# uio-bmi/compairr

Measured on AMD Instinct MI355X. Metric: query sequences/sec for --matrix d=1, 10M-vs-10M CDR3aa, higher is better.
Workload: dtype u64; 1 GPU; synthetic 10M-vs-10M CDR3aa, d=1 substitutions only, V/J matched; queries_total=10000000, queries_this_gpu=10000000, reference_sequences=10000000, matrix_checksum=fc9769626ca2bcf2c84e8473864b8853

## Files before the change

compairr_amd/csrc/query_layout.hip:

```cpp
#include "context.h"
#include "kernels_sliced.h"

#include <hipcub/hipcub.hpp>

#include <algorithm>
#include <atomic>
#include <chrono>
#include <cstdio>
#include <cstdlib>
#include <cstring>
#include <thread>

using namespace cmpr;

namespace {

constexpr uint32_t MAXP = 1 + MAX_CLASS_RES;
constexpr uint32_t FOREIGN_SLICES_LOG2 = 12;

enum : uint32_t { VERR_OFFSETS = 1, VERR_LONG = 2, VERR_REP = 3, VERR_GENE = 4, VERR_COUNT = 5,
                  VERR_RESIDUE = 6, VERR_TOO_LONG = 7, VERR_OFFSETS0 = 8 };

struct SliceTot {
  uint32_t tiles, chunks, small, list;
// ... 55 lines not shown
  SliceTot *tot[MAXP], *pre[MAXP];
  uint32_t  tile0[MAXP], chunk0[MAXP], list0[MAXP], small0[MAXP];
  unsigned long long res0[MAXP];
  uint32_t *tfirst_g;
  uint64_t *h_tmp, *hins_tmp, *hdel_tmp;
  uint32_t *ck_tmp;
  struct QAux *aux;
  TileDesc *tiles;
  Chunk    *chunks;
  TileRef  *tile_refs;
  uint32_t *small_tiles, *chunk_work;
  uint32_t *qres, *qv, *qj, *qck;
  uint64_t *qgh, *qhins, *qhdel;
  uint16_t *qlen;
  QueryRec *qrec;
  uint32_t  ngroups;
  uint32_t  goff[MAX_GROUPS];
  uint32_t  gslices[MAX_GROUPS];
  uint32_t  gslice0[MAX_GROUPS];
  uint32_t  sub2_items;
  uint2    *slice_items;
  uint32_t  nitem_slices;
  uint32_t  cblocks;
  uint32_t *ccnt, *cbase, *cfill, *cnch, *cchpre;
  uint32_t *ccnt_r, *cfill_r, *rbase;
  uint32_t  item_reps;
  uint32_t  item_wg;
  uint32_t  recompute;
  uint32_t  total_on_device;
  uint32_t  zob_lds, zob_words;
  uint32_t  zob_pos_words;
  uint32_t  own_np;
  uint32_t  ctab_lds;
  uint32_t  group_wg, G;
  uint32_t *gbase_w;
  uint32_t  cchunk0;
  cmpr::ItemRec *items;
  cmpr::ResPack *cpk;
  uint32_t           *verr;
  double             *rep_total;
  unsigned long long *alg_bytes;
};

constexpr uint32_t ITEM_WG_MAX = 16384;
constexpr uint32_t ITEM_PAD = 16;
constexpr uint32_t GROUP_WG_MAX = 8192;

enum : uint32_t { LDBG_NO_RANK = 1u << 16, LDBG_NO_ITEM_COUNT = 1u << 17, LDBG_NO_HASH = 1u << 18,
                  LDBG_NO_TOTALS = 1u << 19, LDBG_NO_CLASSKEY = 1u << 20, LDBG_NO_TMP_WRITES = 1u << 21,
                  LDBG_S_NO_REC = 1u << 22, LDBG_S_NO_ITEMS = 1u << 23, LDBG_S_SEQ_REC = 1u << 24,
                  LDBG_S_NO_ITEM_WRITE = 1u << 25, LDBG_S_NO_BASE = 1u << 26 };
#ifdef CMPR_ABLATION
#define LDBG(Q, bit) (((Q).dbg & (bit)) != 0)
#else
#define LDBG(Q, bit) false
#endif

__device__ inline uint64_t total_of(const QL &Q)
{
  return Q.total_on_device ? Q.off[Q.n] : Q.total;
}

__host__ __device__ inline uint32_t work_owner(uint32_t slice, uint32_t pass, uint32_t step)
{
  return (uint32_t)((((uint64_t)slice * 2654435761u + pass * 40503u) >> 7) % step);
}
// ... 119 lines not shown
      } else {
        uint64_t lo = 0, hi = 0;
        for (uint32_t x = 0; x < 16u && at + x < total; x++) {
          const uint64_t r = Q.res[at + x];
          if (x < 8u)
            lo |= r << (8u * x);
          else
            hi |= r << (8u * (x - 8u));
        }
        o.w[k] = make_uint4((uint32_t)lo, (uint32_t)(lo >> 32), (uint32_t)hi, (uint32_t)(hi >> 32));
      }
    }
  }
  return o;
}

template <int NP>
__device__ inline const uint8_t *own_commit(const QL &Q, const OwnPieces<NP> &o, uint64_t b, uint64_t e, uint32_t *mine)
{
  if (!o.fits)
    return Q.res + b;
  const uint64_t a0 = b & ~15ull;
#pragma unroll
  for (uint32_t k = 0; k < (uint32_t)NP; k++)
    if (a0 + 16u * k < e) {
      mine[4 * k + 0] = o.w[k].x;
      mine[4 * k + 1] = o.w[k].y;
      mine[4 * k + 2] = o.w[k].z;
      mine[4 * k + 3] = o.w[k].w;
    }
  return (const uint8_t *)mine + (b - a0);
}

template <typename ZP>
__device__ inline void hashes_of(ZP z, uint32_t A, bool indels, const uint8_t *s, uint32_t L, uint64_t &h,
                                 uint64_t &hins, uint64_t &hdel)
{
  for (uint32_t p = 0; p < L; p++) {
    const uint32_t r = s[p];
    h ^= z[A * p + r];
    if (indels) {
      hins ^= z[A * (p + 1) + r];
      if (p > 0)
        hdel ^= z[A * (p - 1) + r];
    }
  }
}

__device__ inline uint64_t variants_of(const QL &Q, const uint8_t *s, uint32_t L)
{
  const uint64_t A = Q.A;
  uint64_t n = 1;
  if (Q.differences >= 1) {
    n += (A - 1) * L;
    if (Q.indels) {
      if (L > 1) {
        uint64_t runs = 1;
        for (uint32_t p = 1; p < L; p++)
          runs += s[p] != s[p - 1];
        n += runs;
      }
      n += A + (A - 1) * (uint64_t)L;
    }
  }
  if (Q.differences >= 2)
    n += (A - 1) * (A - 1) * (uint64_t)L * (L ? L - 1 : 0) / 2;
  return n;
}

enum : uint32_t { ITEM_SUB = K_SUB, ITEM_INS = K_INS, ITEM_SUB2 = K_SUB2, ITEM_PAIR = 7  };

__device__ inline uint32_t class_base_of(const QL &Q, uint64_t i)
{
  const uint32_t L = (uint32_t)(Q.off[i + 1] - Q.off[i]);
  return class_base(Q.geom.ctab, Q.geom, Q.genes != 0, L, Q.genes ? Q.v[i] : 0u,
                    Q.genes ? Q.j[i] : 0u);
}

template <bool HASH, typename F>
__device__ inline void for_each_item(const QL &Q, const uint32_t *ct, const uint64_t *zt, uint64_t h_of_q,
                                     uint64_t hins_of_q, const uint8_t *s, uint32_t L, uint32_t ck, bool heavy, F f)
{
  const SliceGeom &g = Q.geom;
  const uint32_t K = g.k, A = Q.A;
  if (L == 0 || K == 0 || Q.differences < 1)
    return;
  if (Q.sub2_items) {
    if (heavy && L >= g.c0 + K && L <= RESPACK_MAX)
      for (uint32_t ci = 0; ci < K; ci++) {
        const uint32_t pos = g.c0 + ci, r = s[pos];
        for (uint32_t kp = 1; kp < A; kp++) {
          const uint32_t v = (r + kp) % A;
          const uint32_t key = ck ^ ct[g.off_cr + ci * A + r] ^ ct[g.off_cr + ci * A + v];
          f((key & g.smask) * Q.ngroups + (ci * (A - 1) + kp - 1), 0ull, kp | (pos << 8) | (ITEM_SUB2 << 24));
        }
      }
    return;
  }
  if (Q.pairs) {
    if (heavy) {
      const uint64_t h = HASH ? h_of_q : 0ull;
      for (uint32_t ci = 0; ci < K; ci++) {
        const uint32_t p = class_pos(L, ci, g.c0) & ~1u;
        bool first = true;
        uint32_t key = ck;
        for (uint32_t k = 0; k < K; k++) {
          const uint32_t mk = class_pos(L, k, g.c0);
          if ((mk & ~1u) == p) {
            if (k < ci)
              first = false;
            key ^= ct[g.off_cr + k * A + s[mk]];
          }
        }
        if (first) {
          const uint32_t ra = s[p], rb = p + 1 < L ? (uint32_t)s[p + 1] : A;
          uint64_t w = 0;
          if (HASH) {
            w = h ^ zt[A * p + ra];
            if (p + 1 < L)
              w ^= zt[A * (p + 1) + rb];
          }
          uint32_t fl = 0;
          if (Q.indels && L > 1) {
            if (p == 0 || s[p] != s[p - 1])
              fl |= ITEM_DEL_COUNTS;
            if (p + 1 < L && s[p + 1] != s[p])
              fl |= ITEM_DEL2_COUNTS;
          }
          key ^= pair_part_terms(ct, g, A, L, p, [&](uint32_t pos) -> uint32_t { return s[pos]; });
          f(Q.goff[ci] + (key & g.cmask), w, ra | (rb << 5) | (p << 10) | (ITEM_PAIR << 24) | fl);
        }
      }
    }
    if (!Q.indels)
      return;
    uint32_t base = ck;
    if (heavy)
      for (uint32_t k = 0; k < K; k++)
        base ^= ct[g.off_cr + k * A + s[class_pos(L, k, g.c0)]];
    const uint32_t base_i = base ^ ct[L] ^ ct[L + 1];
    if (!class_is_heavy(g.ctab, g, base_i))
      return;
    const uint64_t hins = HASH ? hins_of_q : 0ull;
    uint64_t P0 = 0, Pp = 0;
    uint64_t cand = 0;
    bool cand_far = false;
    for (uint32_t k = 0; k < K; k++) {
      const uint32_t mk = class_pos(L + 1, k, g.c0);
      if (mk < 64u)
        cand |= 1ull << (mk & ~1u);
      else
        cand_far = true;
    }
    for (uint32_t x = 0; x <= L; x++) {
      if ((x & 1u) == 0 && (x < 64u ? ((cand >> x) & 1ull) != 0 : cand_far)) {
        int ci = -1;
        uint32_t key = base_i;
        for (uint32_t k = 0; k < K; k++) {
          const uint32_t mk = class_pos(L + 1, k, g.c0);
          if ((mk & ~1u) == x) {
            if (ci < 0)
              ci = (int)k;
          } else {
            key ^= ct[g.off_cr + k * A + s[mk < x ? mk : mk - 1]];
          }
        }
        if (ci >= 0) {
          key ^= pair_part_terms(ct, g, A, L + 1, x,
                                 [&](uint32_t pos) -> uint32_t { return s[pos < x ? pos : pos - 1]; });
          uint64_t w = P0 ^ hins ^ Pp;
          if (HASH && x < L)
            w ^= zt[A * (x + 1) + s[x]];
          f(Q.goff[ci] + (key & g.cmask), w,
            (x < L ? (uint32_t)s[x] : A) | ((x > 0 ? (uint32_t)s[x - 1] : 31u) << 5) | (x << 10) | (ITEM_INS << 24));
// ... 18 lines not shown
        if (class_pos(L, k, g.c0) == pos) {
          if (k < ci)
            first = false;
          key ^= ct[g.off_cr + k * A + s[pos]];
        }
      if (first)
        f(Q.goff[ci] + (key & g.cmask), HASH ? h ^ zt[A * pos + s[pos]] : 0ull,
          (uint32_t)s[pos] | (pos << 8) | (ITEM_SUB << 24));
    }
  }
}

template <int MODE>
__device__ inline void layout_mode_assume(const QL &Q)
{
  if (MODE == 3) {
    __builtin_assume(Q.own_np == 3);
    return;
  }
  if (MODE != 0) {
    __builtin_assume(Q.rows != 0);
    __builtin_assume(Q.pairs != 0);
    __builtin_assume(Q.sliced != 0);
    __builtin_assume(Q.pairs2 == 0);
    __builtin_assume(Q.sub2_items == 0);
    __builtin_assume(Q.direct == 0);
    __builtin_assume(Q.route == 0);
    __builtin_assume(Q.differences == 1);
    __builtin_assume(Q.recompute != 0);
    __builtin_assume(Q.wstep <= 1);
    __builtin_assume(Q.dbg == 0);
    __builtin_assume(Q.group_wg == 0);
    __builtin_assume(Q.own_np == 3);
  }
  if (MODE == 1)
    __builtin_assume(Q.indels == 0);
  if (MODE == 2)
    __builtin_assume(Q.indels != 0);
}

template <uint32_t LAYOUT_WG, int MODE>
__global__ void __launch_bounds__(LAYOUT_WG, (LAYOUT_WG == 1024 || MODE == 0) ? 4 : 6)
keys_kernel(const QL Q, uint64_t q0, uint64_t q1, uint32_t row0)
{
  layout_mode_assume<MODE>(Q);
  extern __shared__ double tot_lds[];
  __shared__ uint32_t dest_lds[64];
  const bool lds_tot = Q.n_rep <= 2048;
  uint64_t *const zl = (uint64_t *)(tot_lds + (lds_tot ? Q.n_rep : 0u));
  uint32_t *const ctl = (uint32_t *)(zl + (Q.zob_lds ? Q.zob_words : 0u));
  uint32_t *const ihist = ctl + (Q.ctab_lds ? Q.geom.off_hv : 0u);
  uint32_t *const ghist = ihist + (Q.item_wg ? Q.nitem_slices : 0u);
  constexpr int NP = MODE == 0 ? OWN_NP_MAX : 3;
  const uint32_t own_np = MODE == 0 ? Q.own_np : 3u, own_dw = 4u * own_np + 1u;
  uint32_t *const mine = ghist + (Q.group_wg ? Q.G : 0u) + threadIdx.x * own_dw;
  const uint32_t *const ct = Q.ctab_lds ? ctl : Q.geom.ctab;
  if (lds_tot) {
    for (uint32_t r = threadIdx.x; r < Q.n_rep; r += LAYOUT_WG)
      tot_lds[r] = 0.0;
  }
  if (Q.zob_lds)
    for (uint32_t k = threadIdx.x; k < Q.zob_words; k += LAYOUT_WG)
      zl[k] = Q.zob[k];
  if (Q.ctab_lds)
    for (uint32_t k = threadIdx.x; k < Q.geom.off_hv; k += LAYOUT_WG)
      ctl[k] = Q.geom.ctab[k];
  if (Q.item_wg)
    for (uint32_t k = threadIdx.x; k < Q.nitem_slices; k += LAYOUT_WG)
      ihist[k] = 0;
  if (Q.group_wg)
    for (uint32_t k = threadIdx.x; k < Q.G; k += LAYOUT_WG)
      ghist[k] = 0;
  if (threadIdx.x < 64)
    dest_lds[threadIdx.x] = 0;
  if (Q.total_on_device && blockIdx.x == 0 && threadIdx.x == 0 && q0 == 0 && Q.off[0] != 0)
    atomicCAS(Q.verr, 0u, (uint32_t)VERR_OFFSETS0);
  const uint64_t total = total_of(Q);
  __syncthreads();
  unsigned long long alg = 0;
  uint32_t err_all = 0, Lmax = 0;
  struct Fields {
    uint64_t b, e, cn;
    uint32_t rp, vg, jg;
  };
  auto fetch = [&](uint64_t i) -> Fields {
    Fields f;
    f.b = f.e = 0;
    f.cn = 1;
    f.rp = f.vg = f.jg = 0;
    if (i < q1) {
      f.b = Q.off[i];
      f.e = Q.off[i + 1];
      f.rp = Q.rep[i];
      if (Q.genes) {
        f.vg = Q.v[i];
        f.jg = Q.j[i];
      }
      if (Q.counts)
        f.cn = Q.cnt[i];
    }
    return f;
  };
  const uint64_t stride = (uint64_t)gridDim.x * LAYOUT_WG;
  uint64_t i = q0 + (uint64_t)blockIdx.x * LAYOUT_WG + threadIdx.x;
  Fields cur = fetch(i);
  uint64_t pend_i = ~0ull;
  uint32_t pend_rank = 0;
  for (; i < q1; i += stride) {
    uint32_t err = 0;
    const uint64_t b = cur.b, e = cur.e;
    uint32_t L = 0;
    if (e < b || e > total)
      err = VERR_OFFSETS;
    else if (e - b > 0xffffu)
      err = VERR_LONG;
    else if (e - b > Q.longest)
      err = VERR_TOO_LONG;
    else
      L = (uint32_t)(e - b);
    const uint32_t rp = cur.rp;
    if (!err && rp >= Q.n_rep)
      err = VERR_REP;
    if (!err && Q.genes && (cur.vg >= Q.n_v_max || cur.jg >= Q.n_j_max))
      err = VERR_GENE;
    if (!err && Q.counts && cur.cn < 1)
      err = VERR_COUNT;
    OwnPieces<NP> pieces;
    pieces.fits = false;
    if (!err)
      pieces = own_load<NP>(Q, b, e, total, own_np);
    const Fields nxt = fetch(i + stride);
    const uint8_t *s = err ? Q.res : own_commit(Q, pieces, b, e, mine);
    if (pend_i != ~0ull) {
      Q.rank[pend_i] = pend_rank;
      pend_i = ~0ull;
    }
    const uint64_t cnt_i = cur.cn;
    const uint32_t vg = cur.vg, jg = cur.jg;
    cur = nxt;
    if (!err) {
      bool bad = false;
      for (uint32_t p = 0; p < L; p++)
        bad = bad || s[p] >= Q.A;
      if (bad)
        err = VERR_RESIDUE;
    }
    uint32_t grp_out = 0xffffffffu;
    if (err && !err_all)
      err_all = err;
    if (!err) {
      Lmax = max(Lmax, L);
      const double x = Q.counts ? (double)cnt_i : 1.0;
      if (lds_tot)
        unsafeAtomicAdd(tot_lds + rp, x);
      else
        unsafeAtomicAdd(Q.rep_total + rp, x);
      uint32_t ck = 0;
      bool heavy = false;
      if (Q.sliced && !LDBG(Q, LDBG_NO_CLASSKEY)) {
        ck = class_base(ct, Q.geom, Q.genes != 0, L, vg, jg);
        heavy = Q.geom.k > 0 && class_is_heavy(Q.geom.ctab, Q.geom, ck);
        if (heavy && L > 0)
          for (uint32_t k = 0; k < Q.geom.k; k++)
            ck ^= ct[Q.geom.off_cr + k * Q.A + s[class_pos(L, k, Q.geom.c0)]];
      } else if (Q.sliced)
        ck = (uint32_t)i * 2654435761u;
      if (Q.rows || Q.direct) {
        uint64_t h = 0;
        if (Q.genes) {
          if (Q.zob_lds) {
            const uint64_t *gk = zl + Q.A * Q.zpos;
            h = gk[vg] ^ gk[Q.n_v + jg];
          } else {
            const uint64_t *gk = Q.zob + (uint64_t)Q.A * Q.zpos;
            h = gk[vg] ^ gk[Q.n_v + jg];
          }
        }
        uint64_t hins = h, hdel = h;
        if (Q.zob_lds)
          hashes_of((const uint64_t *)zl, Q.A, Q.indels != 0, s, LDBG(Q, LDBG_NO_HASH) ? 0u : L, h, hins, hdel);
        else
          hashes_of(Q.zob, Q.A, Q.indels != 0, s, LDBG(Q, LDBG_NO_HASH) ? 0u : L, h, hins, hdel);
        if (Q.direct) {
          ck = (uint32_t)(h >> 40);
          Q.h_tmp[i] = h;
        } else if (!LDBG(Q, LDBG_NO_TMP_WRITES)) {
          Q.h_tmp[i] = h;
          if (Q.indels) {
            Q.hins_tmp[i] = hins;
            Q.hdel_tmp[i] = hdel;
          }
          Q.ck_tmp[i] = ck;
        }
      } else if (Q.sub2_items) {
        Q.ck_tmp[i] = ck;
      }
      if (Q.route) {
        unsigned long long mask = 1ull << work_owner(Q.sliced ? (ck & Q.geom.smask) : (ck & DIRECT_OWNER_MASK), 0u, Q.wstep);
        if (Q.ngroups)
          for_each_item<false>(Q, ct, Q.zob, 0ull, 0ull, s, L, ck, heavy, [&](uint32_t k, uint64_t, uint32_t) {
            mask |= 1ull << item_owner(Q, k, Q.wstep);
          });
        if (Q.route == 2u)
          mask = Q.wstep >= 64u ? ~0ull : (1ull << Q.wstep) - 1ull;
        grp_out = (uint32_t)mask;
        Q.rank[i] = (uint32_t)(mask >> 32);
        for (unsigned long long m = mask; m; m &= m - 1ull)
          atomicAdd(&dest_lds[__builtin_ctzll(m)], 1u);
      }
      bool any_item = false;
      if (Q.ngroups && !Q.route && !LDBG(Q, LDBG_NO_ITEM_COUNT))
        for_each_item<false>(Q, ct, Q.zob, 0ull, 0ull, s, L, ck, heavy, [&](uint32_t k, uint64_t, uint32_t) {
          if (item_owned(Q, k)) {
            if (Q.item_wg)
              atomicAdd(&ihist[k], 1u);
            else
              atomicAdd(Q.ccnt_r + (size_t)((uint32_t)(i >> 8) % Q.item_reps) * Q.nitem_slices + k, 1u);
            any_item = true;
          }
        });
      const uint64_t gl = Q.longest - L;
      const uint32_t slice = Q.sliced ? (ck & Q.geom.smask) : (ck & Q.pmask);
      uint64_t bucket = ~0ull;
      if (owned(Q, Q.sliced ? slice : (ck & DIRECT_OWNER_MASK), 0u))
        bucket = Q.sliced ? 2 * (uint64_t)slice + (heavy ? 1 : 0) : slice;
      else if (any_item)
        bucket = 2 * (Q.nslices_real + (((uint32_t)i * 2654435761u) >> (32 - FOREIGN_SLICES_LOG2)));
      if (bucket != ~0ull && !Q.route) {
        const uint32_t g = (uint32_t)(bucket * Q.per_slice + gl);
        grp_out = g;
        pend_rank = (LDBG(Q, LDBG_NO_RANK) ? 0u : Q.group_wg ? atomicAdd(&ghist[g], 1u) : atomicAdd(Q.cnt_g[0] + g, 1u)) |
                    (heavy ? 0x80000000u : 0u);
        pend_i = i;
      }
      if (Q.alg_step <= 1u || work_owner(Q.sliced ? slice : (ck & DIRECT_OWNER_MASK), 0u, Q.alg_step) == Q.alg_first)
        alg += LDBG(Q, LDBG_NO_TOTALS) ? 0ull : (uint64_t)L + 20 + 8 * variants_of(Q, s, L);
    }
    Q.grp[0][i] = grp_out;
  }
  if (pend_i != ~0ull)
    Q.rank[pend_i] = pend_rank;
  if (err_all)
    atomicCAS(Q.verr, 0u, err_all);
  uint32_t m = Lmax;
  for (int o = 32; o > 0; o >>= 1)
    m = max(m, (uint32_t)__shfl_down((int)m, o, WAVE));
  if ((threadIdx.x & 63) == 0 && m)
    atomicMax(Q.verr + 1, m);
  for (int o = 32; o > 0; o >>= 1)
    alg += __shfl_down(alg, o, WAVE);
  if ((threadIdx.x & 63) == 0 && alg)
    atomicAdd(Q.alg_bytes, alg);
  __syncthreads();
  if (lds_tot) {
    for (uint32_t r = threadIdx.x; r < Q.n_rep; r += LAYOUT_WG)
      if (tot_lds[r] != 0.0)
        unsafeAtomicAdd(Q.rep_total + r, tot_lds[r]);
  }
  if (Q.route && threadIdx.x < 64 && dest_lds[threadIdx.x])
    atomicAdd(Q.dest_cnt + threadIdx.x, (unsigned long long)dest_lds[threadIdx.x]);
  if (Q.group_wg) {
    uint32_t *const row = Q.gbase_w + (size_t)(row0 + blockIdx.x) * Q.G;
    for (uint32_t g = threadIdx.x; g < Q.G; g += LAYOUT_WG) {
      const uint32_t cn = ghist[g];
      if (cn)
        row[g] = atomicAdd(Q.cnt_g[0] + g, cn);
    }
  }
  if (Q.item_wg) {
    uint32_t *const row = Q.rbase + (size_t)(row0 + blockIdx.x) * Q.nitem_slices;
    for (uint32_t k = threadIdx.x; k < Q.nitem_slices; k += LAYOUT_WG) {
      const uint32_t cn = ihist[k];
      if (cn)
        row[k] = atomicAdd(Q.ccnt_r + (size_t)k * ITEM_PAD, cn);
// ... 157 lines not shown
              ck.pass |= CHUNK_WITH_ITEMS;
            if (Q.pairs2) {
              uint32_t lmax = 0;
              for (uint32_t t = 0; t < ck.ntiles; t++)
                lmax = max(lmax, Q.tiles[tile_base + k * Q.chunk_tiles + t].len);
              ck.pass |= ((lmax + 1u) / 2u) << 16;
            }
            Q.chunks[Q.chunk0[pi] + at.chunks + k * reps + rp] = ck;
          }
      }
    }
  }
  if (!WRITE) {
    SliceTot t;
    t.tiles = ntiles;
    t.chunks = nchunks;
    t.small = nsmall;
    t.list = nlist;
    t.res = res;
    Q.tot[pi][sl] = t;
  }
  (void)work_lens;
}


template <uint32_t LAYOUT_WG, int MODE>
__global__ void __launch_bounds__(LAYOUT_WG, (LAYOUT_WG == 1024 || MODE == 0) ? 4 : 6)
scatter_kernel(const QL Q, uint64_t q0, uint64_t q1, uint32_t row0)
{
  layout_mode_assume<MODE>(Q);
  extern __shared__ uint64_t scat_lds[];
  uint64_t *const zl = scat_lds;
  uint32_t *const ctl = (uint32_t *)(zl + (Q.zob_lds ? Q.zob_pos_words : 0u));
  uint32_t *const ibase = ctl + (Q.ctab_lds ? Q.geom.off_hv : 0u);
  uint32_t *const gb = ibase + (Q.item_wg ? Q.nitem_slices : 0u);
  constexpr int NP = MODE == 0 ? OWN_NP_MAX : 3;
  const uint32_t own_np = MODE == 0 ? Q.own_np : 3u, own_dw = 4u * own_np + 1u;
  uint32_t *const wave_words = gb + (Q.group_wg ? Q.G : 0u) + (threadIdx.x & ~63u) * own_dw;
  const uint32_t lane = threadIdx.x & 63u;
  uint32_t *const mine = wave_words + lane * own_dw;
  const uint32_t *const ct = Q.ctab_lds ? ctl : Q.geom.ctab;
  const uint64_t *const zt = Q.zob_lds ? zl : Q.zob;
  if (Q.zob_lds)
    for (uint32_t k = threadIdx.x; k < Q.zob_pos_words; k += LAYOUT_WG)
      zl[k] = Q.zob[k];
  if (Q.ctab_lds)
    for (uint32_t k = threadIdx.x; k < Q.geom.off_hv; k += LAYOUT_WG)
      ctl[k] = Q.geom.ctab[k];
  if (Q.group_wg) {
    const uint32_t *const row = Q.gbase_w + (size_t)(row0 + blockIdx.x) * Q.G;
    for (uint32_t g = threadIdx.x; g < Q.G; g += LAYOUT_WG)
      gb[g] = Q.base_g[0][g] + row[g];
  }
  if (Q.zob_lds || Q.ctab_lds || Q.group_wg)
    __syncthreads();
  if (Q.item_wg) {
    const uint32_t *const row = Q.rbase + (size_t)(row0 + blockIdx.x) * Q.nitem_slices;
    for (uint32_t k = threadIdx.x; k < Q.nitem_slices; k += LAYOUT_WG)
      ibase[k] = Q.cbase[k] + row[k];
    __syncthreads();
  }
  const uint64_t total = total_of(Q);
  struct Fields {
    uint64_t b, e;
    uint32_t g, rk;
  };
  const bool want_h = Q.ngroups != 0 && Q.rows, want_ck = Q.ngroups != 0 && (Q.rows || Q.sub2_items);
  auto fetch = [&](uint64_t i) -> Fields {
    Fields f;
    f.b = f.e = 0;
    f.g = 0xffffffffu;
    f.rk = 0;
    if (i < q1) {
      f.g = Q.grp[0][i];
      f.rk = Q.rank[i];
      f.b = Q.off[i];
      f.e = Q.off[i + 1];
    }
    return f;
  };
// ... 5 lines not shown
    uint32_t slot = 0xffffffffu;
    QueryRec qr;
    qr.cnt = 0;
    qr.v = qr.j = qr.rep = qr.len = qr.orig = 0;
    const uint32_t g = cur.g;
    const uint64_t b = cur.b, e = cur.e;
    const uint32_t rk = cur.rk;
    uint32_t gbase = 0, ck = 0;
    uint64_t h_q = 0, hins_q = 0;
    OwnPieces<NP> pieces;
    pieces.fits = false;
    if (g != 0xffffffffu) {
      gbase = LDBG(Q, LDBG_S_NO_BASE) ? 0u : Q.group_wg ? gb[g] : Q.base_g[0][g];
      pieces = own_load<NP>(Q, b, e, total, own_np);
      qr.cnt = Q.counts ? Q.cnt[i] : 1ull;
      qr.v = Q.genes ? Q.v[i] : 0u;
      qr.j = Q.genes ? Q.j[i] : 0u;
      qr.orig = Q.orig ? Q.orig[i] : (uint32_t)i;
      qr.rep = Q.existence ? qr.orig : Q.rep[i];
      if (want_h) {
        h_q = Q.h_tmp[i];
        if (Q.indels)
          hins_q = Q.hins_tmp[i];
      }
      if (want_ck)
        ck = Q.ck_tmp[i];
      if (Q.rec_hash && !want_h)
        h_q = Q.h_tmp[i];
    }
    cur = fetch(i + stride);
    if (g != 0xffffffffu) {
      slot = LDBG(Q, LDBG_S_NO_BASE) ? (uint32_t)i : gbase + (rk & 0x7fffffffu);
      const uint32_t L = (uint32_t)(e - b);
      const uint8_t *s = own_commit(Q, pieces, b, e, mine);
      qr.len = L;
      if (!Q.recompute) {
        QAux a;
        a.h = a.hins = a.hdel = 0;
        a.ck = 0;
        a.src = (uint32_t)i;
        if (Q.rows) {
          a.h = Q.h_tmp[i];
          a.ck = Q.ck_tmp[i];
          if (Q.indels) {
            a.hins = Q.hins_tmp[i];
            a.hdel = Q.hdel_tmp[i];
          }
        } else if (Q.direct) {
          a.h = Q.h_tmp[i];
        } else if (Q.genes) {
          const uint64_t *gk = Q.zob + (uint64_t)Q.A * Q.zpos;
          a.h = gk[Q.v[i]] ^ gk[Q.n_v + Q.j[i]];
        }
        Q.aux[slot] = a;
      }
      if (Q.ngroups != 0 && !LDBG(Q, LDBG_S_NO_ITEMS)) {
        const bool heavy = (rk >> 31) != 0;
        uint64_t hq = 0;
        cmpr::ResPack pk{};
        if (Q.pairs2 && heavy)
          for (uint32_t x = 0; x < L && x < RESPACK_MAX; x++)
            pk.w[x >> 4] |= ((uint32_t)s[x] & 3u) << ((x & 15u) * 2u);
        if (Q.sub2_items && heavy && L <= RESPACK_MAX) {
          if (Q.genes) {
            const uint64_t *gk = Q.zob + (uint64_t)Q.A * Q.zpos;
            hq = gk[qr.v] ^ gk[Q.n_v + qr.j];
          }
          for (uint32_t x = 0; x < L; x++) {
            const uint32_t r = s[x];
            hq ^= Q.zob[Q.A * x + r];
            pk.w[x >> 4] |= (r & 3u) << ((x & 15u) * 2u);
          }
        }
        for_each_item<true>(Q, ct, zt, h_q, hins_q, s, L, ck, heavy, [&](uint32_t k, uint64_t w, uint32_t crp) {
          if (!item_owned(Q, k))
            return;
          uint32_t item;
          if (Q.item_wg) {
            item = atomicAdd(&ibase[k], 1u);
          } else {
            const size_t rk = (size_t)((uint32_t)(i >> 8) % Q.item_reps) * Q.nitem_slices + k;
            item = Q.cbase[k] + Q.rbase[rk] + atomicAdd(Q.cfill_r + rk, 1u);
          }
          if (Q.sub2_items) {
            w = hq;
            Q.cpk[item] = pk;
          } else if (Q.pairs2) {
            Q.cpk[item] = pk;
          }
          ItemRec it;
          it.w = w;
          it.main = slot;
          it.rp = crp;
          if (!LDBG(Q, LDBG_S_NO_ITEM_WRITE))
            Q.items[item] = it;
        });
      }
    }
    if (slot != 0xffffffffu) {
      const uint32_t L = (uint32_t)(e - b);
      if (pieces.fits) {
        const uint32_t o = (uint32_t)(b & 15u), w0 = o >> 2, sh = o & 3u;
        uint32_t lo = mine[w0];
#pragma unroll
        for (uint32_t w = 0; w < 9; w++) {
          const uint32_t hi = mine[w0 + w + 1u];
          const uint32_t d = __builtin_amdgcn_alignbyte(hi, lo, sh);
// ... 909 lines not shown
  c->npasses = 1 + ngroups;
  const uint64_t chunk_tiles =
      c->chunk_tiles > 0 ? (uint64_t)c->chunk_tiles : c->rows ? 64 : 8 * (uint64_t)c->waves_per_block;
  c->chunk_cap = (uint32_t)chunk_tiles;
  const bool mixed_ok = c->sliced && (!c->opt.indels || c->rows);
  const uint64_t n2s = indel_passes ? 2 * nslices : 0;

  struct Range { uint64_t q0, q1; uint32_t grid, row0; };
  std::vector<Range> ranges;
  const bool item_wg = ncs > 0 && ncs <= ITEM_WG_MAX && !routing && c->item_wg != 0;
  const uint64_t zob_words = (uint64_t)A * c->zpos + (c->opt.ignore_genes ? 0 : c->opt.n_v_genes + c->opt.n_j_genes);
  const bool zob_lds = c->layout_zob_lds != 0 && zob_words * sizeof(uint64_t) <= 12288;
  const uint64_t zob_pos_words = (uint64_t)A * c->zpos;
  const bool ctab_lds = c->layout_zob_lds != 0 && c->sliced && c->geom.off_hv <= 2048;
  const size_t ctab_bytes = ctab_lds ? (size_t)c->geom.off_hv * sizeof(uint32_t) : 0;
  const uint32_t own_np_want = std::min<uint32_t>((uint32_t)OWN_NP_MAX, std::max<uint32_t>(3u, (Lcap + 15u + 15u) / 16u));
  const bool group_wg = G <= GROUP_WG_MAX && !routing && c->item_wg != 0;
  const size_t keys_shared = (n_rep <= 2048 ? n_rep * sizeof(double) : 0) + (zob_lds ? zob_words * sizeof(uint64_t) : 0) +
                             ctab_bytes + (item_wg ? (size_t)ncs * sizeof(uint32_t) : 0) + (group_wg ? G * sizeof(uint32_t) : 0);
  const size_t scatter_shared = (zob_lds ? zob_pos_words * sizeof(uint64_t) : 0) + ctab_bytes +
                                (item_wg ? (size_t)ncs * sizeof(uint32_t) : 0) + (group_wg ? G * sizeof(uint32_t) : 0);
  typedef void (*LayoutFn)(const QL, uint64_t, uint64_t, uint32_t);
  static const uint32_t wg_sizes[3] = {256, 512, 1024};
  static const LayoutFn keys_all[4][3] = {{keys_kernel<256, 0>, keys_kernel<512, 0>, keys_kernel<1024, 0>},
                                          {keys_kernel<256, 1>, keys_kernel<512, 1>, keys_kernel<1024, 1>},
                                          {keys_kernel<256, 2>, keys_kernel<512, 2>, keys_kernel<1024, 2>},
                                          {keys_kernel<256, 3>, keys_kernel<512, 3>, keys_kernel<1024, 3>}};
  static const LayoutFn scatter_all[4][3] = {{scatter_kernel<256, 0>, scatter_kernel<512, 0>, scatter_kernel<1024, 0>},
                                             {scatter_kernel<256, 1>, scatter_kernel<512, 1>, scatter_kernel<1024, 1>},
                                             {scatter_kernel<256, 2>, scatter_kernel<512, 2>, scatter_kernel<1024, 2>},
                                             {scatter_kernel<256, 3>, scatter_kernel<512, 3>, scatter_kernel<1024, 3>}};
  const bool recompute_on = Lcap <= 36u && !c->d2pairs && c->layout_recompute != 0;
  const int lmode = (c->rows && pair_rows(c) && !c->d2pairs && !sub2_items && !direct && !routing && wstep <= 1 &&
                     c->opt.differences == 1 && recompute_on && c->debug == 0 && !group_wg)
                        ? (c->opt.indels ? 2 : 1)
                        : own_np_want == 3u ? 3 : 0;
  const LayoutFn *const keys_fns = keys_all[lmode], *const scatter_fns = scatter_all[lmode];
  const uint32_t own_np = lmode ? 3u : own_np_want;
  uint32_t resident = 2048;
  uint32_t LAYOUT_WG = 256;
  size_t keys_lds = 0, scatter_lds = 0;
  LayoutFn keys_fn = keys_fns[0], scatter_fn = scatter_fns[0];
  {
    uint32_t best_waves = 0;
    int bk = 0, bs = 0;
    for (int w = 0; w < 3; w++) {
      const size_t own = (size_t)wg_sizes[w] * (4 * own_np + 1) * sizeof(uint32_t);
      const size_t kl = keys_shared + own, sl = scatter_shared + own;
      if (kl > 160 * 1024 - 512 || sl > 160 * 1024 - 512)
        continue;
      if ((rc = raise_lds_limit(c, (const void *)keys_fns[w], kl))) return rc;
      if ((rc = raise_lds_limit(c, (const void *)scatter_fns[w], sl))) return rc;
      const int ok = occupancy_of(c, (const void *)keys_fns[w], (int)wg_sizes[w], kl);
      const int os = occupancy_of(c, (const void *)scatter_fns[w], (int)wg_sizes[w], sl);
      const uint32_t waves = (uint32_t)std::max(0, std::min(ok, os)) * wg_sizes[w] / WAVE;
      if (waves >= best_waves && waves > 0) {
        best_waves = waves;
        LAYOUT_WG = wg_sizes[w];
        keys_lds = kl;
        scatter_lds = sl;
        keys_fn = keys_fns[w];
        scatter_fn = scatter_fns[w];
        resident = (uint32_t)c->cus * (uint32_t)std::min(ok, os);
        bk = ok;
        bs = os;
      }
    }
    if (best_waves == 0)
      return fail(c, CMPR_EUNSUPPORTED, "the layout kernels' tables do not fit the 160 KiB LDS");
    if (getenv("COMPAIRR_HIP_DEBUG"))
      fprintf(stderr, "compairr_hip: layout kernels: workgroups of %u; keys %zu B of LDS, %d per CU; scatter %zu B, %d; "
                      "grid %u; %llu item counters in %u groups (%s)\n", LAYOUT_WG, keys_lds, bk, scatter_lds, bs,
              resident, (unsigned long long)ncs, ngroups, item_wg ? "per workgroup in LDS" : "replicas in memory");
  }
  {
    const uint64_t min_range = 1u << 18;
    const uint64_t nr = from_host ? std::max<uint64_t>(1, std::min<uint64_t>(4, n / min_range)) : 1;
    static const uint32_t cut4[5] = {0, 30, 60, 86, 100};
    uint32_t row = 0;
    for (uint64_t r = 0; r < nr; r++) {
      Range g;
      g.q0 = nr == 4 ? n * cut4[r] / 100 : n * r / nr;
      g.q1 = nr == 4 ? n * cut4[r + 1] / 100 : n * (r + 1) / nr;
      g.grid = (uint32_t)std::min<uint64_t>(std::max<uint64_t>(1, (g.q1 - g.q0 + LAYOUT_WG - 1) / LAYOUT_WG), resident);
      g.row0 = row;
      row += g.grid;
      ranges.push_back(g);
    }
  }
  const uint64_t item_rows = (uint64_t)ranges.back().row0 + ranges.back().grid;

  ArenaCut cut;
  const size_t o_gcnt = cut.take(G * npass * sizeof(uint32_t));
  const uint32_t item_reps = item_wg ? ITEM_PAD : ncs > 0 && ncs <= 65536 ? 32u : 1u;
  const size_t o_ccnt = cut.take(ncs * sizeof(uint32_t));
  const size_t o_cfill = cut.take(ncs * sizeof(uint32_t));
  const size_t o_ccnt_r = cut.take(ncs * item_reps * sizeof(uint32_t));
  const size_t o_cfill_r = cut.take(item_wg ? 0 : ncs * item_reps * sizeof(uint32_t));
  const size_t o_sibcnt = cut.take(n2s * sizeof(uint32_t));
  const size_t o_sibfill = cut.take(n2s * sizeof(uint32_t));
  const size_t o_alg = cut.take(sizeof(unsigned long long));
  const size_t o_verr = cut.take(2 * sizeof(uint32_t));
  const size_t o_reptot = cut.take((size_t)n_rep * sizeof(double));
  const size_t o_dest = cut.take(2 * 64 * sizeof(unsigned long long));
  const size_t o_sums = cut.take(8 * sizeof(unsigned long long));
  const size_t zero_bytes = cut.used;
// ... 152 lines not shown
  Q.hdel_tmp = (uint64_t *)at(o_hdel);
  Q.ck_tmp = (uint32_t *)at(o_ck);
  Q.alg_bytes = (unsigned long long *)at(o_alg);
  Q.verr = (uint32_t *)at(o_verr);
  Q.rep_total = (double *)at(o_reptot);
  Q.ccnt = (uint32_t *)at(o_ccnt);
  Q.cbase = (uint32_t *)at(o_cbase);
  Q.cfill = (uint32_t *)at(o_cfill);
  Q.ccnt_r = (uint32_t *)at(o_ccnt_r);
  Q.cfill_r = (uint32_t *)at(o_cfill_r);
  Q.rbase = (uint32_t *)at(o_rbase);
  Q.item_reps = item_reps;
  Q.item_wg = item_wg ? 1u : 0u;
  Q.group_wg = group_wg ? 1u : 0u;
  Q.G = (uint32_t)G;
  Q.gbase_w = (uint32_t *)at(o_gbase_w);
  Q.recompute = recompute_on ? 1u : 0u;
  Q.total_on_device = total_on_device ? 1u : 0u;
  Q.cnch = (uint32_t *)at(o_cnch);
  Q.cchpre = (uint32_t *)at(o_cchpre);
  uint32_t *const cpad = (uint32_t *)at(o_cpad);
  uint32_t *const sib_cnt = (uint32_t *)at(o_sibcnt), *const sib_fill = (uint32_t *)at(o_sibfill);
  uint32_t *const sib_nch = (uint32_t *)at(o_sibnch), *const sib_lpre = (uint32_t *)at(o_siblpre);
  uint32_t *const sib_cpre = (uint32_t *)at(o_sibcpre);
  unsigned long long *const sums = (unsigned long long *)at(o_sums);
  void *const cub_tmp = at(o_cub);

  double upload_ms = 0;
  Q.zob_lds = zob_lds ? 1u : 0u;
  Q.zob_words = (uint32_t)zob_words;
  Q.zob_pos_words = (uint32_t)zob_pos_words;
  Q.own_np = own_np;
  Q.ctab_lds = ctab_lds ? 1u : 0u;
  const bool timing = c->layout_timing != 0 && !from_host && c->ev_layout[0] != nullptr;
  c->layout_marks = 0;
#define LAYOUT_MARK(k)                                                      \
  do {                                                                      \
    if (timing) {                                                           \
      HIP_TRY(c, hipEventRecord(c->ev_layout[k], c->stream));               \
      c->layout_marks |= 1u << (k);                                         \
    }                                                                       \
  } while (0)
  if (!from_host) {
    static const uint64_t zero_off1[1] = {0};
    const size_t lds = keys_lds;
    if (n == 0) {
      HIP_TRY(c, hipMemcpyAsync(at(o_off), zero_off1, sizeof(uint64_t), hipMemcpyHostToDevice, c->stream));
    } else {
      if (from_records) {
        const unsigned char *rec = (const unsigned char *)src.d_records;
        hipLaunchKernelGGL(unpack_len_kernel, dim3(blocks_for(n + 1)), dim3(256), 0, c->stream, rec, n,
                           record_bytes, Lcap, (uint16_t *)at(o_len16), Q.verr);
        HIP_TRY(c, hipGetLastError());
        hipcub::TransformInputIterator<unsigned long long, Len16To64, const uint16_t *> it(
            (const uint16_t *)at(o_len16), Len16To64());
        size_t b = cub_bytes;
        HIP_TRY(c, hipcub::DeviceScan::ExclusiveScan(cub_tmp, b, it, (unsigned long long *)at(o_off), hipcub::Sum(),
                                                     0ull, (int)(n + 1), c->stream));
        hipLaunchKernelGGL(unpack_kernel, dim3(blocks_for(n)), dim3(256), 0, c->stream, rec, n, record_bytes,
                           (const uint64_t *)at(o_off), (uint8_t *)at(o_res),
                           c->opt.ignore_genes ? nullptr : (uint32_t *)at(o_v),
                           c->opt.ignore_genes ? nullptr : (uint32_t *)at(o_j), (uint32_t *)at(o_rep),
                           c->opt.ignore_counts ? nullptr : (uint64_t *)at(o_cnt), (uint32_t *)at(o_orig));
        HIP_TRY(c, hipGetLastError());
      }
      LAYOUT_MARK(0);
// ... 590 lines not shown
```

Before: 6.003 billion query sequences/s.

## Stage heavy-class bitmap in LDS, hoist class key, and defer rank atomics

Optionally copies the heavy-bucket bitmap into LDS next to the class table, choosing it when occupancy allows, so heavy-class checks in the keys and scatter kernels read LDS instead of global memory. The class base and its heavy word are computed early in the loop to overlap with residue loads. The per-group rank atomic is deferred one iteration through a pipelined rank_step, and global-address-space loads and atomics are made explicit. In the specialised modes residues are always committed to per-thread LDS words. This costs extra LDS per workgroup, which may lower occupancy, and adds register pressure from the hoisted values.

```diff
diff --git a/compairr_amd/csrc/query_layout.hip b/compairr_amd/csrc/query_layout.hip
--- a/compairr_amd/csrc/query_layout.hip
+++ b/compairr_amd/csrc/query_layout.hip
@@ -111,6 +111,7 @@
   uint32_t  zob_pos_words;
   uint32_t  own_np;
   uint32_t  ctab_lds;
+  uint32_t  hv_lds;
   uint32_t  group_wg, G;
   uint32_t *gbase_w;
   uint32_t  cchunk0;
@@ -296,6 +297,38 @@
   return (const uint8_t *)mine + (b - a0);
 }
 
+__device__ inline const uint8_t *own_commit_lds(const QL &Q, const OwnPieces<3> &o, uint64_t b, uint64_t e, uint32_t *mine)
+{
+  static_assert(4 * OWN_DW >= 36, "the record's residues fit a thread's words");
+  if (!o.fits) {
+    const uint32_t L = (uint32_t)min(e - b, (uint64_t)(4 * OWN_DW));
+    for (uint32_t p = 0; p < L; p++)
+      ((uint8_t *)mine)[p] = Q.res[b + p];
+    return (const uint8_t *)mine;
+  }
+  const uint64_t a0 = b & ~15ull;
+#pragma unroll
+  for (uint32_t k = 0; k < 3; k++)
+    if (a0 + 16u * k < e) {
+      mine[4 * k + 0] = o.w[k].x;
+      mine[4 * k + 1] = o.w[k].y;
+      mine[4 * k + 2] = o.w[k].z;
+      mine[4 * k + 3] = o.w[k].w;
+    }
+  return (const uint8_t *)mine + (b - a0);
+}
+
+__device__ inline uint32_t load_memory_word(const uint32_t *p)
+{
+  return *(const __attribute__((address_space(1))) uint32_t *)p;
+}
+
+__device__ inline uint32_t atomic_inc_memory(uint32_t *p)
+{
+  return __hip_atomic_fetch_add((__attribute__((address_space(1))) uint32_t *)p, 1u, __ATOMIC_RELAXED,
+                                __HIP_MEMORY_SCOPE_AGENT);
+}
+
 template <typename ZP>
 __device__ inline void hashes_of(ZP z, uint32_t A, bool indels, const uint8_t *s, uint32_t L, uint64_t &h,
                                  uint64_t &hins, uint64_t &hdel)
@@ -342,7 +375,7 @@
 }
 
 template <bool HASH, typename F>
-__device__ inline void for_each_item(const QL &Q, const uint32_t *ct, const uint64_t *zt, uint64_t h_of_q,
+__device__ inline void for_each_item(const QL &Q, const uint32_t *ct, bool hv_in_ct, const uint64_t *zt, uint64_t h_of_q,
                                      uint64_t hins_of_q, const uint8_t *s, uint32_t L, uint32_t ck, bool heavy, F f)
 {
   const SliceGeom &g = Q.geom;
@@ -403,7 +436,9 @@
       for (uint32_t k = 0; k < K; k++)
         base ^= ct[g.off_cr + k * A + s[class_pos(L, k, g.c0)]];
     const uint32_t base_i = base ^ ct[L] ^ ct[L + 1];
-    if (!class_is_heavy(g.ctab, g, base_i))
+    const uint32_t hb = base_i >> (32 - HEAVY_BUCKETS_LOG2);
+    const uint32_t hw = hv_in_ct ? ct[g.off_hv + (hb >> 5)] : load_memory_word(g.ctab + g.off_hv + (hb >> 5));
+    if (!((hw >> (hb & 31u)) & 1u))
       return;
     const uint64_t hins = HASH ? hins_of_q : 0ull;
     uint64_t P0 = 0, Pp = 0;
@@ -488,6 +523,8 @@
     __builtin_assume(Q.dbg == 0);
     __builtin_assume(Q.group_wg == 0);
     __builtin_assume(Q.own_np == 3);
+    __builtin_assume(Q.zob_lds != 0);
+    __builtin_assume(Q.ctab_lds != 0);
   }
   if (MODE == 1)
     __builtin_assume(Q.indels == 0);
@@ -505,7 +542,9 @@
   const bool lds_tot = Q.n_rep <= 2048;
   uint64_t *const zl = (uint64_t *)(tot_lds + (lds_tot ? Q.n_rep : 0u));
   uint32_t *const ctl = (uint32_t *)(zl + (Q.zob_lds ? Q.zob_words : 0u));
-  uint32_t *const ihist = ctl + (Q.ctab_lds ? Q.geom.off_hv : 0u);
+  const bool hv_in_ct = Q.ctab_lds && Q.hv_lds;
+  const uint32_t ctl_words = Q.ctab_lds ? Q.geom.off_hv + (hv_in_ct ? HEAVY_WORDS : 0u) : 0u;
+  uint32_t *const ihist = ctl + ctl_words;
   uint32_t *const ghist = ihist + (Q.item_wg ? Q.nitem_slices : 0u);
   constexpr int NP = MODE == 0 ? OWN_NP_MAX : 3;
   const uint32_t own_np = MODE == 0 ? Q.own_np : 3u, own_dw = 4u * own_np + 1u;
@@ -519,7 +558,7 @@
     for (uint32_t k = threadIdx.x; k < Q.zob_words; k += LAYOUT_WG)
       zl[k] = Q.zob[k];
   if (Q.ctab_lds)
-    for (uint32_t k = threadIdx.x; k < Q.geom.off_hv; k += LAYOUT_WG)
+    for (uint32_t k = threadIdx.x; k < ctl_words; k += LAYOUT_WG)
       ctl[k] = Q.geom.ctab[k];
   if (Q.item_wg)
     for (uint32_t k = threadIdx.x; k < Q.nitem_slices; k += LAYOUT_WG)
@@ -531,7 +570,7 @@
     dest_lds[threadIdx.x] = 0;
   if (Q.total_on_device && blockIdx.x == 0 && threadIdx.x == 0 && q0 == 0 && Q.off[0] != 0)
     atomicCAS(Q.verr, 0u, (uint32_t)VERR_OFFSETS0);
-  const uint64_t total = total_of(Q);
+  uint64_t total = total_of(Q);
   __syncthreads();
   unsigned long long alg = 0;
   uint32_t err_all = 0, Lmax = 0;
@@ -559,9 +598,24 @@
   };
   const uint64_t stride = (uint64_t)gridDim.x * LAYOUT_WG;
   uint64_t i = q0 + (uint64_t)blockIdx.x * LAYOUT_WG + threadIdx.x;
+  auto settle = [](Fields &f) {
+    asm volatile("" : "+v"(f.b), "+v"(f.e), "+v"(f.cn), "+v"(f.rp), "+v"(f.vg), "+v"(f.jg));
+  };
   Fields cur = fetch(i);
-  uint64_t pend_i = ~0ull;
-  uint32_t pend_rank = 0;
+  settle(cur);
+  asm volatile("" : "+v"(total));
+  constexpr uint32_t NO_GROUP = 0xffffffffu;
+  uint32_t ask_g = NO_GROUP, got_raw = 0;
+  bool ask_heavy = false, got = false, got_heavy = false;
+  auto rank_step = [&](uint64_t at) {
+    if (got)
+      Q.rank[at - stride] = (got_raw & 0x7fffffffu) | (got_heavy ? 0x80000000u : 0u);
+    got = ask_g != NO_GROUP;
+    got_heavy = ask_heavy;
+    if (got)
+      got_raw = LDBG(Q, LDBG_NO_RANK) ? 0u : Q.group_wg ? atomicAdd(&ghist[ask_g], 1u) : atomic_inc_memory(Q.cnt_g[0] + ask_g);
+    ask_g = NO_GROUP;
+  };
   for (; i < q1; i += stride) {
     uint32_t err = 0;
     const uint64_t b = cur.b, e = cur.e;
@@ -586,14 +640,24 @@
     if (!err)
       pieces = own_load<NP>(Q, b, e, total, own_np);
     const Fields nxt = fetch(i + stride);
-    const uint8_t *s = err ? Q.res : own_commit(Q, pieces, b, e, mine);
-    if (pend_i != ~0ull) {
-      Q.rank[pend_i] = pend_rank;
-      pend_i = ~0ull;
-    }
+    uint32_t ck_base = 0, hv_word = 0;
+    if (!err && Q.sliced && !LDBG(Q, LDBG_NO_CLASSKEY)) {
+      ck_base = class_base(ct, Q.geom, Q.genes != 0, L, cur.vg, cur.jg);
+      if (Q.geom.k > 0) {
+        const uint32_t hw = Q.geom.off_hv + (ck_base >> (32 - HEAVY_BUCKETS_LOG2 + 5));
+        hv_word = hv_in_ct ? ctl[hw] : load_memory_word(Q.geom.ctab + hw);
+      }
+    }
+    const uint8_t *s;
+    if constexpr (MODE != 0)
+      s = err ? (const uint8_t *)mine : own_commit_lds(Q, pieces, b, e, mine);
+    else
+      s = err ? Q.res : own_commit(Q, pieces, b, e, mine);
     const uint64_t cnt_i = cur.cn;
     const uint32_t vg = cur.vg, jg = cur.jg;
     cur = nxt;
+    settle(cur);
+    rank_step(i - stride);
     if (!err) {
       bool bad = false;
       for (uint32_t p = 0; p < L; p++)
@@ -614,8 +678,8 @@
       uint32_t ck = 0;
       bool heavy = false;
       if (Q.sliced && !LDBG(Q, LDBG_NO_CLASSKEY)) {
-        ck = class_base(ct, Q.geom, Q.genes != 0, L, vg, jg);
-        heavy = Q.geom.k > 0 && class_is_heavy(Q.geom.ctab, Q.geom, ck);
+        ck = ck_base;
+        heavy = Q.geom.k > 0 && ((hv_word >> ((ck_base >> (32 - HEAVY_BUCKETS_LOG2)) & 31u)) & 1u) != 0;
         if (heavy && L > 0)
           for (uint32_t k = 0; k < Q.geom.k; k++)
             ck ^= ct[Q.geom.off_cr + k * Q.A + s[class_pos(L, k, Q.geom.c0)]];
@@ -654,7 +718,7 @@
       if (Q.route) {
         unsigned long long mask = 1ull << work_owner(Q.sliced ? (ck & Q.geom.smask) : (ck & DIRECT_OWNER_MASK), 0u, Q.wstep);
         if (Q.ngroups)
-          for_each_item<false>(Q, ct, Q.zob, 0ull, 0ull, s, L, ck, heavy, [&](uint32_t k, uint64_t, uint32_t) {
+          for_each_item<false>(Q, ct, hv_in_ct, Q.zob, 0ull, 0ull, s, L, ck, heavy, [&](uint32_t k, uint64_t, uint32_t) {
             mask |= 1ull << item_owner(Q, k, Q.wstep);
           });
         if (Q.route == 2u)
@@ -666,12 +730,12 @@
       }
       bool any_item = false;
       if (Q.ngroups && !Q.route && !LDBG(Q, LDBG_NO_ITEM_COUNT))
-        for_each_item<false>(Q, ct, Q.zob, 0ull, 0ull, s, L, ck, heavy, [&](uint32_t k, uint64_t, uint32_t) {
+        for_each_item<false>(Q, ct, hv_in_ct, Q.zob, 0ull, 0ull, s, L, ck, heavy, [&](uint32_t k, uint64_t, uint32_t) {
           if (item_owned(Q, k)) {
             if (Q.item_wg)
               atomicAdd(&ihist[k], 1u);
             else
-              atomicAdd(Q.ccnt_r + (size_t)((uint32_t)(i >> 8) % Q.item_reps) * Q.nitem_slices + k, 1u);
+              atomic_inc_memory(Q.ccnt_r + (size_t)((uint32_t)(i >> 8) % Q.item_reps) * Q.nitem_slices + k);
             any_item = true;
           }
         });
@@ -685,17 +749,16 @@
       if (bucket != ~0ull && !Q.route) {
         const uint32_t g = (uint32_t)(bucket * Q.per_slice + gl);
         grp_out = g;
-        pend_rank = (LDBG(Q, LDBG_NO_RANK) ? 0u : Q.group_wg ? atomicAdd(&ghist[g], 1u) : atomicAdd(Q.cnt_g[0] + g, 1u)) |
-                    (heavy ? 0x80000000u : 0u);
-        pend_i = i;
+        ask_g = g;
+        ask_heavy = heavy;
       }
       if (Q.alg_step <= 1u || work_owner(Q.sliced ? slice : (ck & DIRECT_OWNER_MASK), 0u, Q.alg_step) == Q.alg_first)
         alg += LDBG(Q, LDBG_NO_TOTALS) ? 0ull : (uint64_t)L + 20 + 8 * variants_of(Q, s, L);
     }
     Q.grp[0][i] = grp_out;
   }
-  if (pend_i != ~0ull)
-    Q.rank[pend_i] = pend_rank;
+  rank_step(i - stride);
+  rank_step(i);
   if (err_all)
     atomicCAS(Q.verr, 0u, err_all);
   uint32_t m = Lmax;
@@ -919,8 +982,10 @@
   extern __shared__ uint64_t scat_lds[];
   uint64_t *const zl = scat_lds;
   uint32_t *const ctl = (uint32_t *)(zl + (Q.zob_lds ? Q.zob_pos_words : 0u));
-  uint32_t *const ibase = ctl + (Q.ctab_lds ? Q.geom.off_hv : 0u);
-  uint32_t *const gb = ibase + (Q.item_wg ? Q.nitem_slices : 0u);
+  const bool hv_in_ct = Q.ctab_lds && Q.hv_lds && Q.indels;
+  const uint32_t ctl_words = Q.ctab_lds ? Q.geom.off_hv + (hv_in_ct ? HEAVY_WORDS : 0u) : 0u;
+  uint32_t *const ibase = ctl + ctl_words;
+  uint32_t *const gb =ibase + (Q.item_wg ? Q.nitem_slices : 0u);
   constexpr int NP = MODE == 0 ? OWN_NP_MAX : 3;
   const uint32_t own_np = MODE == 0 ? Q.own_np : 3u, own_dw = 4u * own_np + 1u;
   uint32_t *const wave_words = gb + (Q.group_wg ? Q.G : 0u) + (threadIdx.x & ~63u) * own_dw;
@@ -932,7 +997,7 @@
     for (uint32_t k = threadIdx.x; k < Q.zob_pos_words; k += LAYOUT_WG)
       zl[k] = Q.zob[k];
   if (Q.ctab_lds)
-    for (uint32_t k = threadIdx.x; k < Q.geom.off_hv; k += LAYOUT_WG)
+    for (uint32_t k = threadIdx.x; k < ctl_words; k += LAYOUT_WG)
       ctl[k] = Q.geom.ctab[k];
   if (Q.group_wg) {
     const uint32_t *const row = Q.gbase_w + (size_t)(row0 + blockIdx.x) * Q.G;
@@ -1004,7 +1069,11 @@
     if (g != 0xffffffffu) {
       slot = LDBG(Q, LDBG_S_NO_BASE) ? (uint32_t)i : gbase + (rk & 0x7fffffffu);
       const uint32_t L = (uint32_t)(e - b);
-      const uint8_t *s = own_commit(Q, pieces, b, e, mine);
+      const uint8_t *s;
+      if constexpr (MODE != 0)
+        s = own_commit_lds(Q, pieces, b, e, mine);
+      else
+        s = own_commit(Q, pieces, b, e, mine);
       qr.len = L;
       if (!Q.recompute) {
         QAux a;
@@ -1044,7 +1113,7 @@
             pk.w[x >> 4] |= (r & 3u) << ((x & 15u) * 2u);
           }
         }
-        for_each_item<true>(Q, ct, zt, h_q, hins_q, s, L, ck, heavy, [&](uint32_t k, uint64_t w, uint32_t crp) {
+        for_each_item<true>(Q, ct, hv_in_ct, zt, h_q, hins_q, s, L, ck, heavy, [&](uint32_t k, uint64_t w, uint32_t crp) {
           if (!item_owned(Q, k))
             return;
           uint32_t item;
@@ -2020,7 +2089,7 @@
                                              {scatter_kernel<256, 3>, scatter_kernel<512, 3>, scatter_kernel<1024, 3>}};
   const bool recompute_on = Lcap <= 36u && !c->d2pairs && c->layout_recompute != 0;
   const int lmode = (c->rows && pair_rows(c) && !c->d2pairs && !sub2_items && !direct && !routing && wstep <= 1 &&
-                     c->opt.differences == 1 && recompute_on && c->debug == 0 && !group_wg)
+                     c->opt.differences == 1 && recompute_on && c->debug == 0 && !group_wg && zob_lds && ctab_lds)
                         ? (c->opt.indels ? 2 : 1)
                         : own_np_want == 3u ? 3 : 0;
   const LayoutFn *const keys_fns = keys_all[lmode], *const scatter_fns = scatter_all[lmode];
@@ -2028,38 +2097,44 @@
   uint32_t resident = 2048;
   uint32_t LAYOUT_WG = 256;
   size_t keys_lds = 0, scatter_lds = 0;
+  bool hv_lds = false;
+  const size_t hv_bytes = HEAVY_WORDS * sizeof(uint32_t);
   LayoutFn keys_fn = keys_fns[0], scatter_fn = scatter_fns[0];
   {
     uint32_t best_waves = 0;
     int bk = 0, bs = 0;
-    for (int w = 0; w < 3; w++) {
-      const size_t own = (size_t)wg_sizes[w] * (4 * own_np + 1) * sizeof(uint32_t);
-      const size_t kl = keys_shared + own, sl = scatter_shared + own;
-      if (kl > 160 * 1024 - 512 || sl > 160 * 1024 - 512)
-        continue;
-      if ((rc = raise_lds_limit(c, (const void *)keys_fns[w], kl))) return rc;
-      if ((rc = raise_lds_limit(c, (const void *)scatter_fns[w], sl))) return rc;
-      const int ok = occupancy_of(c, (const void *)keys_fns[w], (int)wg_sizes[w], kl);
-      const int os = occupancy_of(c, (const void *)scatter_fns[w], (int)wg_sizes[w], sl);
-      const uint32_t waves = (uint32_t)std::max(0, std::min(ok, os)) * wg_sizes[w] / WAVE;
-      if (waves >= best_waves && waves > 0) {
-        best_waves = waves;
-        LAYOUT_WG = wg_sizes[w];
-        keys_lds = kl;
-        scatter_lds = sl;
-        keys_fn = keys_fns[w];
-        scatter_fn = scatter_fns[w];
-        resident = (uint32_t)c->cus * (uint32_t)std::min(ok, os);
-        bk = ok;
-        bs = os;
-      }
-    }
+    for (int hv = ctab_lds ? 1 : 0; hv >= 0; hv--)
+      for (int w = 0; w < 3; w++) {
+        const size_t own = (size_t)wg_sizes[w] * (4 * own_np + 1) * sizeof(uint32_t);
+        const size_t kl = keys_shared + own + (hv ? hv_bytes : 0);
+        const size_t sl = scatter_shared + own + (hv && c->opt.indels ? hv_bytes : 0);
+        if (kl > 160 * 1024 - 512 || sl > 160 * 1024 - 512)
+          continue;
+        if ((rc = raise_lds_limit(c, (const void *)keys_fns[w], kl))) return rc;
+        if ((rc = raise_lds_limit(c, (const void *)scatter_fns[w], sl))) return rc;
+        const int ok = occupancy_of(c, (const void *)keys_fns[w], (int)wg_sizes[w], kl);
+        const int os = occupancy_of(c, (const void *)scatter_fns[w], (int)wg_sizes[w], sl);
+        const uint32_t waves = (uint32_t)std::max(0, std::min(ok, os)) * wg_sizes[w] / WAVE;
+        if (waves > 0 && (waves > best_waves || (waves == best_waves && hv == (hv_lds ? 1 : 0)))) {
+          best_waves = waves;
+          hv_lds = hv != 0;
+          LAYOUT_WG = wg_sizes[w];
+          keys_lds = kl;
+          scatter_lds = sl;
+          keys_fn = keys_fns[w];
+          scatter_fn = scatter_fns[w];
+          resident = (uint32_t)c->cus * (uint32_t)std::min(ok, os);
+          bk = ok;
+          bs = os;
+        }
+      }
     if (best_waves == 0)
       return fail(c, CMPR_EUNSUPPORTED, "the layout kernels' tables do not fit the 160 KiB LDS");
     if (getenv("COMPAIRR_HIP_DEBUG"))
       fprintf(stderr, "compairr_hip: layout kernels: workgroups of %u; keys %zu B of LDS, %d per CU; scatter %zu B, %d; "
-                      "grid %u; %llu item counters in %u groups (%s)\n", LAYOUT_WG, keys_lds, bk, scatter_lds, bs,
-              resident, (unsigned long long)ncs, ngroups, item_wg ? "per workgroup in LDS" : "replicas in memory");
+                      "grid %u; %llu item counters in %u groups (%s); heavy bitmap in %s\n", LAYOUT_WG, keys_lds, bk,
+              scatter_lds, bs, resident, (unsigned long long)ncs, ngroups,
+              item_wg ? "per workgroup in LDS" : "replicas in memory", hv_lds ? "LDS" : "memory");
   }
   {
     const uint64_t min_range = 1u << 18;
@@ -2278,6 +2353,7 @@
   Q.zob_pos_words = (uint32_t)zob_pos_words;
   Q.own_np = own_np;
   Q.ctab_lds = ctab_lds ? 1u : 0u;
+  Q.hv_lds = hv_lds ? 1u : 0u;
   const bool timing = c->layout_timing != 0 && !from_host && c->ev_layout[0] != nullptr;
   c->layout_marks = 0;
 #define LAYOUT_MARK(k)                                                      \
```

Result: slower. 5.778 billion query sequences/s (-3.7%).
